# ksadov/FREUD

Hardware: AMD Instinct MI355X
Metric: SAE train activations/sec (d=384 dict 8x) (higher is better)
Workload: dtype bf16; 1 GPU; Whisper-tiny d=384 dict 8x (n=3072) L1 SAE train step, M=65536 rows/GPU/step, RAdam+cosine, x bfloat16 resident in HBM (BASELINE configs[1]); rows_per_gpu=65536, d_model=384, n_dict=3072, parallelism=dp1, dp=none

## Files before the change

### freud_amd/csrc/engine.hip

```cpp
#include <hip/hip_runtime.h>
#include <math.h>
#include <stdarg.h>
#include <stdio.h>
#include <string.h>

#include <algorithm>
#include <utility>
#include <vector>

#include "../../include/freud_sae.h"
#include "l1_kernels.h"
#include "gemm256.h"
#include "gemm256s.h"
#include "gemm256_fp8.h"
#include "l1_fp8.h"
#include "dp_kernels.h"
#include "p2p_exchange.h"
#include <rccl/rccl.h>
#include <mutex>
#include <unistd.h>

static thread_local bool g_force_gemm128 = false;
static thread_local bool g_no_stream = false;
static thread_local int g_device = 0;
// ... 67 lines not shown
  KID_PREP_X,
  KID_ENC_FWD,
  KID_DEC_FWD,
  KID_FWD_FUSED,
  KID_DPRE,
  KID_DW,
  KID_BWD_FUSED,
  KID_REDUCE,
  KID_OPT,
  KID_TK_ENC,
  KID_TK_SELECT,
  KID_TK_DECODE,
  KID_TK_DDENSE,
  KID_TK_DWD,
  KID_TK_DWE,
  KID_TK_DSAE,
  KID_TK_AUX,
  KID_EXCHANGE,
  KID_STATS_XCHG,
  KID_STEP_TOTAL,
  KID_COUNT
};
static const char* kKernelNames[KID_COUNT] = {"prep_w", "prep_x", "enc_fwd_gemm", "dec_fwd_gemm", "fwd_fused_gemm", "dpre_gemm",
                                              "dw_gemm", "bwd_fused_gemm", "reduce_grads", "clip_adam", "topk_enc_gemm", "topk_select",
                                              "topk_decode", "topk_ddense_gemm", "topk_dwdec_gemm", "topk_dwenc_gemm",
                                              "topk_dsaein_colsum", "topk_auxk_backward", "dp_exchange", "dp_stats_exchange",
                                              "fwd_bwd_total"};
constexpr int EV_RING = 64;

struct EvRing {
  hipEvent_t beg[EV_RING], end[EV_RING];
  int n = 0;
};

enum LastCall { LAST_FWD_BF16 = 0, LAST_FWD_E32, LAST_SEARCH, LAST_STATS };

struct sae_ctx {
  sae_config cfg;
  int d, n, d_p, n_p;
  int64_t max_rows_p;
  int64_t nW;
  int64_t nparams;
  float *P = nullptr, *Mom = nullptr, *Var = nullptr;
  float* G = nullptr;
  bf16_t *Wb = nullptr, *Wt = nullptr;
  bool fp8 = false;
  bool fp8_bwd = false;
  unsigned char* dxh8 = nullptr;
  int row_pad = 128;
  unsigned char *x8 = nullptr, *c8 = nullptr, *W8 = nullptr, *W8t = nullptr;
  float *scal8 = nullptr, *x8_part = nullptr;
  bool use_fused_fwd = false;
  int fwd_variant = 2;
  bf16_t *xb = nullptr, *c = nullptr, *dxh = nullptr, *dpre = nullptr;
  bf16_t *dxhT = nullptr, *xT = nullptr;
  float *slab = nullptr, *db_part = nullptr, *l1_part = nullptr, *sq_part = nullptr, *scal = nullptr;
  double* gn_part = nullptr;
  float* cn_part = nullptr;
  bool cn_valid = false;
  bool wb_valid = false;
  float* cnorm = nullptr;
  bool wn_pending = false, wn_fwd_seen = false;
  sae_grad_ready_fn grad_ready = nullptr;
  void* grad_ready_user = nullptr;
  int dw_chunk_rows = 0;
  int dw_chunk_splits = 1;
  int dw_col_chunks = 1;
  int dw_col_splits = 1;
  float* cnt_part = nullptr;
  int gn_blocks = 0;
  bool step_fused_call = false;
  bool gn_valid = false;
  bool metrics_fresh = false;
  const bf16_t* xb_cur = nullptr;
  unsigned int* masked = nullptr;
  int dw_splits = 1;
  int dw_tail_tiles = 0, dw_tail_pieces = 0;
  float* dw_tail = nullptr;
  int bwd_splits = 1;
  int bwd_range_splits = 1;
  bool use_fused_bwd = false;
  bool topk = false;
  int k = 0, k_aux_cap = 0;
  int64_t rows_per_file = 0;
  double dead_threshold = 1e300;
  bf16_t *We_b = nullptr, *Wd_b = nullptr, *xs = nullptr, *pre = nullptr, *dense = nullptr, *aux_dense = nullptr;
  bf16_t *de_b = nullptr, *dh_b = nullptr;
  float *e = nullptr, *dh = nullptr, *e2_part = nullptr, *a2_part = nullptr, *dbd_part = nullptr, *ds_part = nullptr, *tkf = nullptr;
  int *top_idx = nullptr, *aux_idx = nullptr, *tk = nullptr;
  bf16_t *top_vals = nullptr, *aux_vals = nullptr, *multi_vals = nullptr;
  unsigned short* tile_max = nullptr;
  unsigned char* sel_flag = nullptr;
  bool dense_valid = false;
  bool multi_dense_valid = false;
  float* be_r = nullptr;
  int slab_splits = 1;
  bool aux_compact = false;
  int *tkd = nullptr, *dead_cols = nullptr, *vec_rank = nullptr;
  unsigned char* vec_bits = nullptr;
  bf16_t* Wdd_b = nullptr;
  float* aux_dbe_part = nullptr;
  int* dead_hint = nullptr;
  double* tv_part = nullptr;
  long long* nfsf = nullptr;
  long long* dbe_fx = nullptr;
  bool topk_sparse_da = false;
// ... 342 lines not shown
    return fail(SAE_ERR_INVALID, "Invalid precision: %d, must be SAE_PREC_BF16, SAE_PREC_FP8 or SAE_PREC_FP8_BWD", cfg->precision);
  if (cfg->precision != SAE_PREC_BF16 && cfg->variant != SAE_VARIANT_L1)
    return fail(SAE_ERR_INVALID, "fp8 encoder / decoder GEMMs exist for the L1 variant only");

  sae_ctx* c = new sae_ctx();
  c->cfg = *cfg;
  c->d = cfg->d_model;
  c->n = cfg->n_dict;
  c->fp8 = cfg->precision != SAE_PREC_BF16;
  c->fp8_bwd = cfg->precision == SAE_PREC_FP8_BWD;
  const int pad = c->fp8 ? 256 : 128;
  c->row_pad = pad;
  c->d_p = (int)round_up(c->d, pad);
  c->n_p = (int)round_up(c->n, pad);
  c->max_rows_p = round_up(cfg->max_rows, pad);
  c->nW = (int64_t)c->d_p * c->n_p;
  c->nparams = c->nW + c->n_p;
  c->topk = cfg->variant == SAE_VARIANT_TOPK;
  if (const char* fg = getenv("FREUD_P2P_FINEGRAINED")) c->finegrained = atoi(fg) == 1;
  const int64_t Mp = c->max_rows_p;
  if (c->topk) {
    int rc_tk = topk_create(c, Mp);
    if (rc_tk) {
      sae_destroy(c);
      return rc_tk;
    }
    *out = c;
    return SAE_OK;
  }
  g_force_gemm128 = cfg->force_gemm128 == 1;
  c->no_stream = g_no_stream = cfg->debug_flags == 86 || (getenv("FREUD_GEMM_STREAM") && atoi(getenv("FREUD_GEMM_STREAM")) == 0);
  c->dw_splits = choose_splits(c->d_p / 128, c->n_p / 128, 2 * Mp / 64);
  if (const char* ov = getenv("FREUD_DW_SPLITS")) {
    const int v = atoi(ov);
    if (v >= 1 && v <= 64) c->dw_splits = v;
  }
  c->dw_chunk_rows = c->d_p >= 1024 ? 512 : c->d_p;
  if (!g_force_gemm128 && c->d_p % 256 == 0 && c->n_p % 256 == 0 && (c->d_p / 256) * (c->n_p / 256) >= 256 && !getenv("FREUD_DW_SPLITS") &&
      c->cfg.debug_flags != 81) {
    gemm_tail_plan((c->d_p / 256) * (c->n_p / 256), (int)(2 * Mp / 64), c->dw_tail_tiles, c->dw_tail_pieces);
    if ((c->d_p / 256) * (c->n_p / 256) % 256 == 0) c->dw_tail_tiles = c->dw_tail_pieces = -1;
  }
  c->dw_chunk_splits = choose_splits(c->dw_chunk_rows / 128, c->n_p / 128, 2 * Mp / 64);
  if (c->d_p >= 1024 && c->n_p % 256 == 0)
    for (int q = 4; q >= 2; --q)
      if ((c->n_p / 256) % q == 0) {
        c->dw_col_chunks = q;
        break;
      }
  c->dw_col_splits = choose_splits(c->d_p / 128, c->n_p / 128 / c->dw_col_chunks, 2 * Mp / 64);
  c->use_fused_bwd = (c->d_p == BF_D) && cfg->force_generic != 1 && !c->fp8;
  c->use_fused_fwd = (c->d_p == FF_D) && cfg->force_generic != 1 && !c->fp8;
  if (const char* fv = getenv("FREUD_FWD")) c->fwd_variant = atoi(fv) == 1 ? 1 : 2;
  c->bwd_splits = fused_bwd_splits(c->n_p / BF_BN, (int)(Mp / BF_BM), c->n_p);
  c->bwd_range_splits = c->bwd_splits;
  for (int r = 2; r <= 4; ++r)
    if ((c->n_p / BF_BN) % r == 0) {
      const int sp = fused_bwd_splits(c->n_p / BF_BN / r, (int)(Mp / BF_BM), c->n_p / r);
      if (sp > c->bwd_range_splits) c->bwd_range_splits = sp;
    }
  int slab_splits = c->use_fused_bwd ? (c->bwd_range_splits > c->dw_splits ? c->bwd_range_splits : c->dw_splits) : c->dw_splits;
  if (c->use_fused_bwd && c->cfg.debug_flags != 83 && !getenv("FREUD_BWD_UNIFORM")) {
    const int ntiles = c->n_p / BF_BN, cus = 256;
    const int m = (32 * ntiles + cus - 1) / cus, grid = (32 * ntiles + m - 1) / m;
    int pmax = 1;
    for (int j = 0; j < ntiles; ++j) pmax = bal_pieces(j, m) > pmax ? bal_pieces(j, m) : pmax;
    const int steps = (int)(Mp / BF_BM), q = (steps + 31) / 32;
    const double slab_steps = (double)c->n_p * BF_D * 8.0 / 4.0e12 / 1.43e-6;
    const double cost_bal = (double)m * q + 5.0 + (32 % m ? 3.5 : 0.0) + (32.0 / m + (32 % m ? 1.0 : 0.0)) * slab_steps;
    const int sp = c->bwd_splits, rounds = (ntiles * sp + 255) / 256;
    const double cost_uni = rounds * ((double)((steps + sp - 1) / sp) + 5.0) + sp * slab_steps;
    if (cost_bal < cost_uni * 0.995 && pmax <= 64 && grid <= 4096) {
      c->bal_m = m;
      c->bal_grid = grid;
      if (pmax > slab_splits) slab_splits = pmax;
      std::vector<int> order(grid);
      for (int k = 0; k < grid; ++k) order[k] = k;
      std::stable_sort(order.begin(), order.end(), [m](int a_, int b_) { return (a_ * m) % 32 < (b_ * m) % 32; });
      std::vector<short> map(grid);
      int pos = 0;
      for (int x = 0; x < 8; ++x) {
        const int len = grid / 8 + (x < grid % 8 ? 1 : 0);
        for (int i = 0; i < len; ++i) map[8 * i + x] = (short)order[pos++];
      }
      hipError_t e_ = hipMalloc((void**)&c->bal_map, (size_t)grid * 2);
      if (e_ == hipSuccess) e_ = hipMemcpy(c->bal_map, map.data(), (size_t)grid * 2, hipMemcpyHostToDevice);
      if (e_ != hipSuccess) {
        int rc_ = fail(SAE_ERR_HIP, "balanced backward: workgroup table: %s", hipGetErrorString(e_));
        sae_destroy(c);
        return rc_;
      }
    }
  }
  {
    const int64_t need = (int64_t)(c->dw_chunk_splits > c->dw_col_splits ? c->dw_chunk_splits : c->dw_col_splits);
    if (need > slab_splits) slab_splits = (int)need;
  }
  const int64_t db_rows = (Mp / 128) > 64 ? (Mp / 128) : 64;

#define ALLOC(ptr, bytes)                                   \
  do {                                                      \
    hipError_t e_ = hipMalloc((void**)&(ptr), (bytes));     \
    if (e_ != hipSuccess) {                                 \
      int rc_ = fail(SAE_ERR_HIP, "hipMalloc(%lld bytes) for %s failed: %s", (long long)(bytes), #ptr, \
                     hipGetErrorString(e_));                \
      sae_destroy(c);                                       \
// ... 889 lines not shown
template <typename T>
static int forward_impl(sae_ctx* c, const T* x, int64_t M, int64_t Mp, hipStream_t s, bool need_backward) {
  const int d = c->d, d_p = c->d_p, n_p = c->n_p;
  const float alpha = (float)c->cfg.recon_alpha;
  float* W = c->P;
  float* b = c->P + c->nW;

  ev_begin(c, KID_PREP_W, s);
  prep_weights_l1(c, s);
  if (c->fp8) hipLaunchKernelGGL(fp8_cast_w_kernel, dim3(n_p / 64, d_p / 64), dim3(256), 0, s, W, c->W8, c->W8t, d_p, n_p);
  ev_end(c, KID_PREP_W, s);

  ev_begin(c, KID_PREP_X, s);
  const bool alias_x = c->use_fused_fwd && sizeof(T) == 2 && x_dtype_is_bf16<T>() && d == d_p && M == Mp &&
                       (reinterpret_cast<uintptr_t>(x) & 15) == 0;
  c->xb_cur = alias_x ? reinterpret_cast<const bf16_t*>(x) : c->xb;
  if (!alias_x) {
    const int grid = launch_prep_x(c, x, M, Mp, s);
    if (!c->use_fused_fwd) {
      const double* gs = (need_backward && c->dp_world > 0) ? c->stats : nullptr;
      if (gs && c->dist) HIP_TRY(hipStreamWaitEvent(s, c->ev_stats, 0));
      hipLaunchKernelGGL(finalize_count_kernel, dim3(1), dim3(256), 0, s, c->masked, grid, c->scal, M, d, alpha, gs);
    }
  }
  if (c->fp8) {
    const int sgrid = (int)((Mp / 4) < 1024 ? (Mp / 4) : 1024);
    hipLaunchKernelGGL(fp8_x_stats_kernel, dim3(sgrid), dim3(256), 0, s, c->xb, Mp, d_p, c->x8_part);
    hipLaunchKernelGGL(fp8_scales_kernel, dim3(1), dim3(256), 0, s, c->x8_part, sgrid, b, c->n, c->scal8);
    const int64_t n8 = Mp * (d_p / 8);
    hipLaunchKernelGGL(fp8_quant_x_kernel, dim3(grid_for(n8, 2048)), dim3(256), 0, s, c->xb, c->x8, n8, c->scal8);
  }
  ev_end(c, KID_PREP_X, s);

  int rc;
  if (c->use_fused_fwd) {
    const int lds = FF_LDS_BYTES;
    FwdFusedArgs a{};
    a.xb = c->xb_cur; a.x = x; a.Wt = c->Wt; a.bias = b; a.cnt_part = c->cnt_part; a.c = c->c; a.dxh = c->dxh;
    a.l1_part = c->l1_part; a.sq_part = c->sq_part; a.M = M; a.d = d; a.n_p = n_p; a.ntiles = n_p / FF_BN;
    a.c_rows = c->max_rows_p;
    const int full_wgs = (int)(M / FF_BM), all_wgs = (int)(Mp / FF_BM);
    auto launch = [&](auto kern, int blocks, int block_offset) -> int {
      LDS_ATTR(kern, 160 * 1024, g_device);
      a.block_offset = block_offset;
      hipLaunchKernelGGL(kern, dim3(blocks), dim3(256), lds, s, a);
      return SAE_OK;
    };
    ev_begin(c, KID_FWD_FUSED, s);
    int rcl = SAE_OK;
    if (full_wgs > 0 && c->cfg.debug_flags == 65 && c->fwd_variant == 1) {
      a.stamps = reinterpret_cast<unsigned long long*>(c->dpre);
      rcl = launch(fwd_fused_d384_kernel<T, false, true>, full_wgs, 0);
    } else if (c->fwd_variant == 2) {
      if (full_wgs > 0 && c->cfg.debug_flags == 65) {
        a.stamps = reinterpret_cast<unsigned long long*>(c->dpre);
        rcl = launch(fwd_fused2_d384_kernel<T, false, true>, full_wgs, 0);
      } else if (full_wgs > 0) rcl = launch(fwd_fused2_d384_kernel<T, false>, full_wgs, 0);
      if (!rcl && all_wgs > full_wgs) rcl = launch(fwd_fused2_d384_kernel<T, true>, all_wgs - full_wgs, full_wgs);
      if (rcl) return rcl;
      ev_end(c, KID_FWD_FUSED, s);
      HIP_TRY(hipGetLastError());
      return SAE_OK;
    } else if (full_wgs > 0) {
      rcl = launch(fwd_fused_d384_kernel<T, false, false>, full_wgs, 0);
    }
    if (!rcl && all_wgs > full_wgs) rcl = launch(fwd_fused_d384_kernel<T, true, false>, all_wgs - full_wgs, full_wgs);
    if (rcl) return rcl;
    ev_end(c, KID_FWD_FUSED, s);
    HIP_TRY(hipGetLastError());
    return SAE_OK;
  }
  if (c->fp8) {
    {
      Gemm8Args g{};
      g.A = c->x8; g.B = c->W8t; g.lda = d_p; g.ldb = d_p;
      g.nbm = (int)(Mp / 256); g.nbn = n_p / 256; g.ktiles = d_p / 128;
      EpiEnc8 e{};
      e.c = c->c; e.c8 = c->c8; e.bias = b; e.scal8 = c->scal8; e.l1_part = c->l1_part; e.M = M; e.n_p = n_p; e.nbn = n_p / 128;
      if (gemm8_streams<EpiEnc8>(g)) HIP_TRY(hipMemsetAsync(c->l1_part, 0, (size_t)(Mp / 128) * (n_p / 128) * 4, s));
      ev_begin(c, KID_ENC_FWD, s);
      rc = launch_gemm8(g, e, s);
      ev_end(c, KID_ENC_FWD, s);
      if (rc) return rc;
    }
    {
      Gemm8Args g{};
      g.A = c->c8; g.B = c->W8; g.lda = n_p; g.ldb = n_p;
      g.nbm = (int)(Mp / 256); g.nbn = d_p / 256; g.ktiles = n_p / 128;
      EpiDec<T> e{};
      e.x = x; e.dxh = c->dxh; e.scal = c->scal; e.sq_part = c->sq_part; e.M = M; e.d = d; e.d_p = d_p; e.nbn = d_p / 128;
      e.vec_all = (M == Mp && d == d_p && d % 4 == 0 && (reinterpret_cast<uintptr_t>(x) % (4 * sizeof(T))) == 0) ? 1 : 0;
      e.vscale = c->scal8 + S8_INV_DEC;
      ev_begin(c, KID_DEC_FWD, s);
      rc = launch_gemm8(g, e, s);
      ev_end(c, KID_DEC_FWD, s);
      if (rc) return rc;
    }
    if (need_backward && c->dxhT) {
      hipLaunchKernelGGL(transpose_bf16_kernel, dim3((unsigned)(Mp / 64), d_p / 64), dim3(256), 0, s, c->dxh, c->dxhT, Mp, d_p);
      hipLaunchKernelGGL(transpose_bf16_kernel, dim3((unsigned)(Mp / 64), d_p / 64), dim3(256), 0, s, c->xb_cur, c->xT, Mp, d_p);
      HIP_TRY(hipGetLastError());
    }
    return SAE_OK;
  }
  rc = launch_encoder<T>(c, enc_gemm_args(c, c->xb_cur, Mp), M, s);
  if (rc) return rc;
  {
    GemmArgs g{};
    g.A0 = c->c; g.B0 = c->Wb; g.lda = n_p; g.ldb = n_p;
    g.nbm = (int)(Mp / 128); g.nbn = d_p / 128; g.ktiles0 = g.ktiles = n_p / 64; g.splits = 1;
// ... 1447 lines not shown
```

### freud_amd/csrc/fwd_fused2.h

```cpp
#pragma once
#include "fwd_fused.h"

typedef __attribute__((ext_vector_type(2))) float f32x2_t;

template <typename T, bool PAD, bool STAMP = false>
__global__ __launch_bounds__(256, 1) void fwd_fused2_d384_kernel(FwdFusedArgs a) {
  extern __shared__ __attribute__((aligned(16))) char smem[];
  const int t = threadIdx.x, lane = t & 63, w = t >> 6;
  const int arow = lane & 31, ah = lane >> 5;
  const int wg = blockIdx.x + a.block_offset;
  const int64_t m0 = (int64_t)wg * FF_BM + 32 * w;
  const int64_t mrow = m0 + arow;
  const bool row_ok = mrow < a.M;
  char* cst = smem + FF_RING_BYTES;
  float* bias_s = reinterpret_cast<float*>(smem + FF_FIXED_LDS);
  unsigned long long clk_k0 = 0, clk_t0 = 0, clk_r0 = 0, clk_t1 = 0;
  if (STAMP) clk_k0 = __builtin_amdgcn_s_memtime();

  typedef __attribute__((ext_vector_type(2))) unsigned short us2_t;
  constexpr unsigned MASK_BITS2 = std::is_same<T, bf16_t>::value ? 0xBF80BF80u : 0xBC00BC00u;
  constexpr bool SCAN_EARLY = !PAD && std::is_same<T, bf16_t>::value;
  bool wany_early = false;

  bf16x8 xfrag[24];
  unsigned voff_t[6], loff_t[6];
#pragma unroll
  for (int i = 0; i < 6; ++i) {
    const int inst = w + 4 * i, sub = inst >> 3, row = 4 * (inst & 7) + (lane >> 4), pc = lane & 15;
    const int ch = pc ^ (((row & 3) << 2) | ((row >> 2) & 3));
    voff_t[i] = (unsigned)(row * (FF_D * 2) + (sub * 16 + ch) * 16);
    loff_t[i] = (unsigned)__builtin_amdgcn_readfirstlane(sub * 8192 + (inst & 7) * 1024);
  }
  typedef __attribute__((address_space(3))) char* lptr_t;
  const unsigned smem_base = (unsigned)(uintptr_t)(lptr_t)smem;
  auto dma_pair = [&](int p, int jt, int st) {
    const bf16_t* src = a.Wt + (int64_t)jt * FF_BN * FF_D;
    const unsigned dst = smem_base + st * FF_WT_BYTES;
    glds16_x2(src, src, voff_t[2 * p], voff_t[2 * p + 1], (unsigned)__builtin_amdgcn_readfirstlane((int)(dst + loff_t[2 * p])),
              (unsigned)__builtin_amdgcn_readfirstlane((int)(dst + loff_t[2 * p + 1])));
  };
  auto dma_one = [&](int k, int jt, int st) {
    const bf16_t* src = a.Wt + (int64_t)jt * FF_BN * FF_D;
    glds16(src, voff_t[k], (unsigned)__builtin_amdgcn_readfirstlane((int)(smem_base + st * FF_WT_BYTES + loff_t[k])));
  };
  const int last = a.ntiles - 1;
#pragma unroll
  for (int q = 0; q < 3; ++q)
#pragma unroll
    for (int p = 0; p < 3; ++p) dma_pair(p, q <= last ? q : last, q);
  static_assert(2 * FF_BN == 64, "one 4-byte piece per lane of wave 0");
  if (w == 0) glds4(a.bias, (unsigned)(lane * 4), (unsigned)__builtin_amdgcn_readfirstlane((int)(smem_base + FF_FIXED_LDS)));
  {
    const bf16_t* xp = a.xb + mrow * FF_D + 8 * ah;
#pragma unroll
    for (int kk = 0; kk < 24; ++kk) xfrag[kk] = *reinterpret_cast<const bf16x8*>(xp + 16 * kk);
  }
  for (int i = t; i < FF_WT_BYTES / 16; i += 256) reinterpret_cast<u32x4*>(smem + 3 * FF_WT_BYTES)[i] = u32x4{0u, 0u, 0u, 0u};
  for (int i = t; i < FF_CST_BYTES / 16; i += 256) reinterpret_cast<u32x4*>(cst)[i] = u32x4{0u, 0u, 0u, 0u};

  f32x16 acc[12];
#pragma unroll
  for (int i = 0; i < 12; ++i)
#pragma unroll
    for (int r = 0; r < 16; ++r) acc[i][r] = 0.f;

  if (SCAN_EARLY) {
    us2_t mz = {0xFFFFu, 0xFFFFu};
#pragma unroll
    for (int kk = 0; kk < 24; ++kk) {
      const u32x4 xw = __builtin_bit_cast(u32x4, xfrag[kk]);
#pragma unroll
      for (int c = 0; c < 4; ++c) mz = __builtin_elementwise_min(mz, __builtin_bit_cast(us2_t, xw[c] ^ MASK_BITS2));
    }
    wany_early = __builtin_amdgcn_ballot_w64((mz[0] == 0) | (mz[1] == 0)) != 0ull;
  }
#pragma unroll
  for (int kk = 0; kk < 24; ++kk) asm volatile("" : "+v"(xfrag[kk]));
  asm volatile("s_waitcnt vmcnt(0)" ::: "memory");
  __syncthreads();

  int roff[8];
#pragma unroll
  for (int i = 0; i < 8; ++i) roff[i] = dual_off(arow, 2 * i + ah);
  int aoff0[6], aoff1[6];
  {
    const int g = (lane >> 4) & 1, q = (lane & 15) >> 2, p = lane & 3;
#pragma unroll
    for (int f = 0; f < 6; ++f) {
      const int ks = f / 3, dt = 3 * w + f % 3;
      const int col = 32 * (dt & 3) + 16 * g + 4 * p;
      const int r0 = 4 * ah + q, r1 = r0 + 8;
      const int base = (dt >> 2) * 8192 + ks * 4096;
      aoff0[f] = base + dual_off(r0, col >> 3) + (col & 7) * 2;
      aoff1[f] = base + dual_off(r1, col >> 3) + (col & 7) * 2;
    }
  }
  typedef __attribute__((ext_vector_type(8))) short s16x8;
  auto tr_pair = [&](const char* p0, const char* p1) -> bf16x8 {
    const s16x4 lo = __builtin_amdgcn_ds_read_tr16_b64_v4i16(LDS_PTR(s16x4, p0));
    const s16x4 hi = __builtin_amdgcn_ds_read_tr16_b64_v4i16(LDS_PTR(s16x4, p1));
    const s16x8 v = __builtin_shufflevector(lo, hi, 0, 1, 2, 3, 4, 5, 6, 7);
    return __builtin_bit_cast(bf16x8, v);
  };
  auto swz = [](int row) { return (row & 7) ^ ((row >> 1) & 1) ^ ((row >> 4) & 1); };
  int boff[4];
#pragma unroll
  for (int i = 0; i < 4; ++i) boff[i] = arow * 128 + (((4 * (i >> 1) + 2 * (i & 1) + ah) ^ swz(arow)) << 4);
  const int wrow = w * 4096;
  const int drow_l = lane >> 3, dch = lane & 7;
  int doff0, doff1;
  {
    const int tl = dch >> 2, s = (dch & 3) >> 1, u = dch & 1;
    doff0 = drow_l * 128 + (((4 * tl + 2 * s + 0) ^ swz(drow_l)) << 4) + 8 * u;
    doff1 = drow_l * 128 + (((4 * tl + 2 * s + 1) ^ swz(drow_l)) << 4) + 8 * u;
  }
  auto dpiece = [](int off, int p) { return (p & 2) ? (off ^ 16) : off; };
  bf16_t* cdrain = a.c + (m0 + drow_l) * a.n_p + dch * 8;

  float l1_acc = 0.f;

  f32x16 Sn;
#pragma unroll
  for (int r = 0; r < 16; ++r) Sn[r] = 0.f;
#pragma unroll
  for (int kk = 0; kk < 24; ++kk) {
    const bf16x8 fa = *reinterpret_cast<const bf16x8*>(smem + (kk >> 3) * 8192 + roff[kk & 7]);
    Sn = __builtin_amdgcn_mfma_f32_32x32x16_bf16(fa, xfrag[kk], Sn, 0, 0, 0);
  }

  constexpr int RING = 8;
  const char *rlo[8], *rhi[8];
#pragma unroll
  for (int i = 0; i < 8; ++i) {
// ... 93 lines not shown
      if (i == 41 || i == 45) dma_one((i - 41) / 4, jt, SLOT_DMA);
      if (i == 1 || i == 5 || i == 9 || i == 13) dma_one(2 + (i - 1) / 4, j + 2 <= last ? j + 2 : last, (PH + 2) & 3);
      if ((PH & 1) == 0 && i == 46 && w == 0) {
        const int jb = j + 2 <= a.ntiles - 2 ? j + 2 : a.ntiles - 2;
        glds4(a.bias + (int64_t)jb * FF_BN, (unsigned)(lane * 4),
              (unsigned)__builtin_amdgcn_readfirstlane((int)(smem_base + FF_FIXED_LDS + ((j + 2) & (FF_BIAS_RING_TILES - 1)) * FF_BN * 4)));
      }
      if (i >= 4 && i <= 35) {
        const int p = (i - 4) >> 2, ph = (i - 4) & 3, e0 = 2 * p;
        if (ph == 0) {
          se_u = __builtin_bit_cast(unsigned, __builtin_convertvector(f32x2_t{S[e0], S[e0 + 1]}, bf16x2));
        } else if (ph == 1) {
          se_t0 = __uint_as_float(se_u << 16) + bq[e0 >> 2][e0 & 3];
          se_t1 = __uint_as_float(se_u & 0xFFFF0000u);
        } else if (ph == 2) {
          se_t1 = se_t1 + bq[e0 >> 2][(e0 & 3) + 1];
          se_t0 = fmaxf(se_t0, 0.f);
          se_t1 = fmaxf(se_t1, 0.f);
          if (PAD) { se_t0 = row_ok ? se_t0 : 0.f; se_t1 = row_ok ? se_t1 : 0.f; }
        } else {
          asm volatile("v_add_f32 %0, %0, %1\n\tv_add_f32 %0, %0, %2" : "+v"(l1_it) : "v"(se_t0), "v"(se_t1));
          cw[e0 & 7] = (bf16_t)se_t0;
          cw[(e0 & 7) + 1] = (bf16_t)se_t1;
          if ((e0 & 7) == 6)
            *reinterpret_cast<bf16x8*>(cst + PB_W * 16384 + wrow + boff[2 * HF_W + (e0 >> 3)]) = cw;
        }
      }
      if (i == 29 || i == 33) {
        const int p = 2 * (PH & 1) + (i == 33);
        const uint2 lo = *reinterpret_cast<const uint2*>(cst_r + p * 1024 + dpiece(doff0, p));
        const uint2 hi = *reinterpret_cast<const uint2*>(cst_r + p * 1024 + dpiece(doff1, p));
        dr[i == 33] = u32x4{lo.x, lo.y, hi.x, hi.y};
      }
      if (i == 37 || i == 42) {
        const int p = 2 * (PH & 1) + (i == 42);
        __builtin_nontemporal_store(dr[i == 42], reinterpret_cast<u32x4*>(dst_pair + (int64_t)(8 * p) * dst_rstride));
      }
      __builtin_amdgcn_sched_barrier(0);
      if ((i & 1) == 0) {
        const int m = i / 2, ks = m / 12, mb = (m % 12) / 3, dtl = m % 3;
        acc[4 * dtl + mb] = __builtin_amdgcn_mfma_f32_32x32x16_bf16(Afr[3 * ks + dtl], Bq[(4 * ks + mb) & 3], acc[4 * dtl + mb], 0, 0, 0);
      } else if (i == 1) {
        f32x16 zero;
#pragma unroll
        for (int r = 0; r < 16; ++r) zero[r] = 0.f;
        Snxt = __builtin_amdgcn_mfma_f32_32x32x16_bf16(ring[0], xfrag[0], zero, 0, 0, 0);
      } else {
        Snxt = __builtin_amdgcn_mfma_f32_32x32x16_bf16(ring[(i / 2) % RING], xfrag[i / 2], Snxt, 0, 0, 0);
      }
      __builtin_amdgcn_sched_barrier(0);
    });
    l1_acc += l1_it + 0.0f;
  };
  if (STAMP) { clk_t0 = __builtin_amdgcn_s_memtime(); clk_r0 = __builtin_amdgcn_s_memrealtime(); }
  for (int j4 = 0; j4 < a.ntiles; j4 += 4) {
    body(std::integral_constant<int, 0>{}, j4);
    body(std::integral_constant<int, 1>{}, j4 + 1);
    body(std::integral_constant<int, 2>{}, j4 + 2);
    body(std::integral_constant<int, 3>{}, j4 + 3);
  }
  if (STAMP) {
    const unsigned long long t1 = __builtin_amdgcn_s_memtime(), r1 = __builtin_amdgcn_s_memrealtime();
    clk_t1 = t1;
    if (lane == 0) {
      unsigned long long* o = a.stamps + ((int64_t)wg * 4 + w) * 8;
      o[0] = o[1] = o[2] = 0; o[3] = (unsigned long long)a.ntiles; o[4] = t1 - clk_t0; o[5] = r1 - clk_r0; o[6] = clk_t0 - clk_k0;
    }
  }
  Bq[2] = dec_b(1, 1, 2);
#pragma unroll
  for (int m = 0; m < 24; ++m) {
    if (m == 3 || m == 4 || m == 5) Afr[m] = dec_a(3, m);
    if (m % 3 == 0 && m / 3 + 3 <= 7) Bq[(m / 3 + 3) & 3] = dec_b(1, 1, m / 3 + 3);
    __builtin_amdgcn_sched_barrier(0);
    const int ks = m / 12, mb = (m % 12) / 3, dtl = m % 3;
    acc[4 * dtl + mb] = __builtin_amdgcn_mfma_f32_32x32x16_bf16(Afr[3 * ks + dtl], Bq[(4 * ks + mb) & 3], acc[4 * dtl + mb], 0, 0, 0);
    __builtin_amdgcn_sched_barrier(0);
  }
  {
    const char* cst_r = cst + (((a.ntiles >> 1) - 1) & 1) * 16384 + wrow;
#pragma unroll
    for (int p = 0; p < 4; ++p) {
      const uint2 lo = *reinterpret_cast<const uint2*>(cst_r + p * 1024 + dpiece(doff0, p));
      const uint2 hi = *reinterpret_cast<const uint2*>(cst_r + p * 1024 + dpiece(doff1, p));
      __builtin_nontemporal_store(u32x4{lo.x, lo.y, hi.x, hi.y},
                                  reinterpret_cast<u32x4*>(cdrain + (int64_t)(8 * p) * a.n_p + 64 * ((a.ntiles >> 1) - 1)));
    }
  }
  __builtin_amdgcn_sched_barrier(0);
  asm volatile("s_waitcnt vmcnt(4) lgkmcnt(0)" ::: "memory");
  __builtin_amdgcn_s_barrier();
  __builtin_amdgcn_sched_barrier(0);

  unsigned long long clk_e0 = 0, clk_e1 = 0, clk_e2 = 0;
  if (STAMP) clk_e0 = __builtin_amdgcn_s_memtime();
  float sq = 0.f, plain = 0.f, nmask = 0.f;
  float msq = 0.f;
  f32x2_t plain2 = {0.f, 0.f};
  typedef __attribute__((ext_vector_type(4))) T Tx4;
  const bool vec_ok = (a.d == FF_D) && ((reinterpret_cast<uintptr_t>(a.x) & (sizeof(T) * 4 - 1)) == 0);
  constexpr int FF_DXH_PITCH = FF_D * 2 + 16;
  static_assert(128 * FF_DXH_PITCH <= FF_FIXED_LDS, "the dx_hat staging must fit the idle LDS");
  char* stg = smem;
  constexpr bool X_VIA_LDS = !PAD && sizeof(T) == 2;
  constexpr bool X_FROM_FRAGS = X_VIA_LDS && std::is_same<T, bf16_t>::value;
  unsigned* mflag = reinterpret_cast<unsigned*>(smem + FF_FIXED_LDS + 64);
  bool blk_masked = true;
  if (X_FROM_FRAGS && vec_ok && reinterpret_cast<const void*>(a.x) == reinterpret_cast<const void*>(a.xb)) {
    char* srow_w = stg + (32 * w + arow) * FF_DXH_PITCH + 16 * ah;
    us2_t mz = {0xFFFFu, 0xFFFFu};
#pragma unroll
    for (int kk = 0; kk < 24; ++kk) {
      *reinterpret_cast<bf16x8*>(srow_w + 32 * kk) = xfrag[kk];
      if (!SCAN_EARLY) {
        const u32x4 xw = __builtin_bit_cast(u32x4, xfrag[kk]);
#pragma unroll
        for (int c = 0; c < 4; ++c) mz = __builtin_elementwise_min(mz, __builtin_bit_cast(us2_t, xw[c] ^ MASK_BITS2));
      }
    }
    const bool wany = SCAN_EARLY ? wany_early : __builtin_amdgcn_ballot_w64((mz[0] == 0) | (mz[1] == 0)) != 0ull;
    if (lane == 0) mflag[w] = wany ? 1u : 0u;
    __syncthreads();
    const u32x4 f = *reinterpret_cast<const u32x4*>(mflag);
    blk_masked = (f[0] | f[1] | f[2] | f[3]) != 0u;
  } else
  if (X_VIA_LDS && vec_ok) {
    const char* xblk = reinterpret_cast<const char*>(reinterpret_cast<const T*>(a.x) + m0 * FF_D);
    us2_t mz = {0xFFFFu, 0xFFFFu};
#pragma unroll
    for (int p0 = 0; p0 < 24; p0 += 4) {
      u32x4 xr[4];
#pragma unroll
      for (int pc = 0; pc < 4; ++pc) xr[pc] = *reinterpret_cast<const u32x4*>(xblk + (p0 + pc) * 1024 + lane * 16);
#pragma unroll
      for (int pc = 0; pc < 4; ++pc) {
        const int off = (p0 + pc) * 1024 + lane * 16, r = off / (FF_D * 2), cb = off - r * (FF_D * 2);
        *reinterpret_cast<u32x4*>(stg + (32 * w + r) * FF_DXH_PITCH + cb) = xr[pc];
#pragma unroll
        for (int c = 0; c < 4; ++c) mz = __builtin_elementwise_min(mz, __builtin_bit_cast(us2_t, xr[pc][c] ^ MASK_BITS2));
      }
    }
    const bool wany = __builtin_amdgcn_ballot_w64((mz[0] == 0) | (mz[1] == 0)) != 0ull;
    if (lane == 0) mflag[w] = wany ? 1u : 0u;
    __syncthreads();
    const u32x4 f = *reinterpret_cast<const u32x4*>(mflag);
    blk_masked = (f[0] | f[1] | f[2] | f[3]) != 0u;
  }
  if (STAMP) clk_e1 = __builtin_amdgcn_s_memtime();
  auto residual = [&](auto notest_tag) {
  constexpr bool NOTEST = decltype(notest_tag)::value;
  constexpr bool FENCE = NOTEST && X_VIA_LDS;
  constexpr bool PIPE = FENCE && std::is_same<T, bf16_t>::value;
  Tx4 xq[2][4];
  auto xload = [&](int g, Tx4 (&dst)[4]) {
    const char* sr = stg + (32 * (g / 3) + arow) * FF_DXH_PITCH + (96 * w + 32 * (g % 3) + 4 * ah) * 2;
#pragma unroll
    for (int k = 0; k < 4; ++k) dst[k] = *reinterpret_cast<const Tx4*>(sr + 16 * k);
  };
  if constexpr (PIPE) xload(0, xq[0]);
#pragma unroll
  for (int mb = 0; mb < 4; ++mb) {
    const int64_t grow = (int64_t)wg * FF_BM + 32 * mb + arow;
    const bool ok = !PAD || grow < a.M;
    const float rmask = ok ? 1.f : 0.f;
    const T* xrow = reinterpret_cast<const T*>(a.x) + (ok ? grow : a.M - 1) * a.d;
    char* srow = stg + (32 * mb + arow) * FF_DXH_PITCH;
#pragma unroll
    for (int dtl = 0; dtl < 3; ++dtl) {
      const int dbase = 96 * w + 32 * dtl + 4 * ah;
      if (NOTEST || vec_ok) {
        const int g = 3 * mb + dtl;
        if constexpr (FENCE) {
          if (g > 0) __builtin_amdgcn_sched_barrier(0);
          if (PIPE && g + 1 < 12) xload(g + 1, xq[(g + 1) & 1]);
        }
        Tx4 xv[4];
#pragma unroll
        for (int k = 0; k < 4; ++k)
          xv[k] = PIPE ? xq[g & 1][k]
                       : (X_VIA_LDS ? *reinterpret_cast<const Tx4*>(srow + (dbase + 8 * k) * 2) : *reinterpret_cast<const Tx4*>(xrow + dbase + 8 * k));
        if (!PAD) {
          if constexpr (NOTEST && X_VIA_LDS) {
            if constexpr (std::is_same<T, bf16_t>::value) {
              uint2 ow[4];
#pragma unroll
              for (int k = 0; k < 4; ++k) {
                const uint2 xw = __builtin_bit_cast(uint2, xv[k]);
#pragma unroll
                for (int pp = 0; pp < 2; ++pp) {
                  const unsigned xd = pp ? xw.y : xw.x;
                  const unsigned rb = __builtin_bit_cast(unsigned, __builtin_convertvector(
                      f32x2_t{acc[4 * dtl + mb][4 * k + 2 * pp], acc[4 * dtl + mb][4 * k + 2 * pp + 1]}, bf16x2));
                  const f32x2_t rf = {__uint_as_float(rb << 16), __uint_as_float(rb & 0xFFFF0000u)};
                  const f32x2_t xf = {__uint_as_float(xd << 16), __uint_as_float(xd & 0xFFFF0000u)};
                  f32x2_t e2, d2;
                  asm("v_pk_add_f32 %0, %1, %2 neg_lo:[0,1] neg_hi:[0,1]" : "=v"(e2) : "v"(rf), "v"(xf));
                  asm("v_pk_fma_f32 %0, %1, %1, %0" : "+v"(plain2) : "v"(e2));
                  asm("v_pk_add_f32 %0, %1, %1" : "=v"(d2) : "v"(e2));
                  const unsigned ob = __builtin_bit_cast(unsigned, __builtin_convertvector(d2, bf16x2));
                  if (pp) ow[k].y = ob; else ow[k].x = ob;
                }
// ... 26 lines not shown
              const float e = bf16_round(acc[4 * dtl + mb][4 * k + q]) - xf;
              const bool mk = xf == -1.0f;
              const float em = mk ? e : 0.0f, ek = mk ? 0.0f : e;
              plain = __builtin_fmaf(e, e, plain);
              msq = __builtin_fmaf(em, em, msq);
              nm_i += mk ? 1u : 0u;
              o[k][q] = (bf16_t)(ek + ek);
            }
          nmask += (float)nm_i;
#pragma unroll
          for (int k = 0; k < 4; ++k) *reinterpret_cast<bf16x4*>(srow + (dbase + 8 * k) * 2) = o[k];
          continue;
        }
#pragma unroll
        for (int k = 0; k < 4; ++k) {
          bf16x4 o;
#pragma unroll
          for (int q = 0; q < 4; ++q) {
            const float xf = (float)xv[k][q];
            const float e = bf16_round(acc[4 * dtl + mb][4 * k + q]) - xf;
            const float e2 = e * e;
            plain += rmask * e2;
            const float keep = (xf != -1.0f) ? rmask : 0.f;
            nmask += rmask - keep;
            sq += keep * e2;
            o[q] = (bf16_t)(keep * (e * 2.0f));
          }
          *reinterpret_cast<bf16x4*>(srow + (dbase + 8 * k) * 2) = o;
        }
      } else {
#pragma unroll
        for (int k = 0; k < 4; ++k) {
          bf16x4 o;
#pragma unroll
          for (int q = 0; q < 4; ++q) {
            const int dd = dbase + 8 * k + q;
            const bool valid = dd < a.d;
            const float xf = (float)xrow[valid ? dd : a.d - 1];
            const float e = bf16_round(acc[4 * dtl + mb][4 * k + q]) - xf;
            const float e2 = valid ? e * e : 0.f;
            plain += rmask * e2;
            const float keep = (valid && xf != -1.0f) ? rmask : 0.f;
            nmask += (valid ? rmask : 0.f) - keep;
            sq += keep * e2;
            o[q] = (bf16_t)(keep * (e * 2.0f));
          }
          *reinterpret_cast<bf16x4*>(srow + (dbase + 8 * k) * 2) = o;
        }
      }
    }
  }
  };
  if (X_VIA_LDS && vec_ok && !blk_masked) residual(std::true_type{}); else residual(std::false_type{});
  if (STAMP) clk_e2 = __builtin_amdgcn_s_memtime();
  __syncthreads();
  {
    char* gblk = reinterpret_cast<char*>(a.dxh + m0 * FF_D);
#pragma unroll
    for (int pc = 0; pc < 24; ++pc) {
      const int off = pc * 1024 + lane * 16, r = off / (FF_D * 2), cb = off - r * (FF_D * 2);
      *reinterpret_cast<u32x4*>(gblk + off) = *reinterpret_cast<const u32x4*>(stg + (32 * w + r) * FF_DXH_PITCH + cb);
    }
  }
  plain += plain2[0] + plain2[1];
  if (!PAD && vec_ok) sq = plain - msq;
  float* red = reinterpret_cast<float*>(smem + FF_FIXED_LDS);
  {
    const float v0 = wave_sum(l1_acc), v1 = wave_sum(sq), v2 = wave_sum(plain), v3 = wave_sum(nmask);
    if (lane == 0) *reinterpret_cast<f32x4*>(red + 4 * w) = f32x4{v0, v1, v2, v3};
  }
  lds_barrier();
  const float l1s = ((red[0] + red[4]) + red[8]) + red[12];
  const float sqs = ((red[1] + red[5]) + red[9]) + red[13];
  const float pls = ((red[2] + red[6]) + red[10]) + red[14];
  const float nms = ((red[3] + red[7]) + red[11]) + red[15];
  if (STAMP && lane == 0) {
    unsigned long long* o = a.stamps + ((int64_t)wg * 4 + w) * 8;
    const unsigned long long te = __builtin_amdgcn_s_memtime();
    o[7] = te - clk_k0;
    o[0] = clk_e0 - clk_t1; o[1] = clk_e1 - clk_e0; o[2] = clk_e2 - clk_e1;
#ifdef FF2_WAITSTAMP
    o[0] = ws_vm; o[1] = ws_bar; o[2] = ws_gap;
#endif
  }
  if (t == 0) {
    a.cnt_part[wg] = nms;
    a.l1_part[wg] = l1s;
    a.sq_part[2 * wg] = sqs;
    a.sq_part[2 * wg + 1] = pls;
  }
}
```

Before: 120.5 million activations/s.

## Make fused d384 forward kernel persistent with early prefetch of next block's x

Changes the bf16 fused forward kernel into a persistent grid of about one workgroup per CU that walks row blocks with a stride, instead of launching one workgroup per 128-row block. During the epilogue of each block it issues the x-fragment loads for the next block, overlapping global loads with the residual computation. It also moves the reduction scratch to a separate LDS offset and swaps some __syncthreads for LDS-only barriers. This removes per-workgroup launch and prologue cost, but it re-streams the W tiles for every block, raises register pressure from the prefetched fragments, and may unbalance the tail.

Measured after the change: 120.6 million activations/s (median of 2 runs). About the same (+0.1%).

```diff
diff --git a/freud_amd/csrc/engine.hip b/freud_amd/csrc/engine.hip
--- a/freud_amd/csrc/engine.hip
+++ b/freud_amd/csrc/engine.hip
@@ -143,6 +143,8 @@
   float *scal8 = nullptr, *x8_part = nullptr;
   bool use_fused_fwd = false;
   int fwd_variant = 2;
+  int fwd_cus = 256;
+  int fwd_wgs = 0;
   bf16_t *xb = nullptr, *c = nullptr, *dxh = nullptr, *dpre = nullptr;
   bf16_t *dxhT = nullptr, *xT = nullptr;
   float *slab = nullptr, *db_part = nullptr, *l1_part = nullptr, *sq_part = nullptr, *scal = nullptr;
@@ -591,6 +593,11 @@
   c->use_fused_bwd = (c->d_p == BF_D) && cfg->force_generic != 1 && !c->fp8;
   c->use_fused_fwd = (c->d_p == FF_D) && cfg->force_generic != 1 && !c->fp8;
   if (const char* fv = getenv("FREUD_FWD")) c->fwd_variant = atoi(fv) == 1 ? 1 : 2;
+  {
+    int cus = 0;
+    if (hipDeviceGetAttribute(&cus, hipDeviceAttributeMultiprocessorCount, cfg->device_id) == hipSuccess && cus > 0) c->fwd_cus = cus;
+    if (const char* fw = getenv("FREUD_FWD_WGS")) c->fwd_wgs = atoi(fw) > 0 ? atoi(fw) : 0;
+  }
   c->bwd_splits = fused_bwd_splits(c->n_p / BF_BN, (int)(Mp / BF_BM), c->n_p);
   c->bwd_range_splits = c->bwd_splits;
   for (int r = 2; r <= 4; ++r)
@@ -1586,10 +1593,13 @@
       a.stamps = reinterpret_cast<unsigned long long*>(c->dpre);
       rcl = launch(fwd_fused_d384_kernel<T, false, true>, full_wgs, 0);
     } else if (c->fwd_variant == 2) {
+      int G = full_wgs < c->fwd_cus ? full_wgs : c->fwd_cus;
+      if (G < full_wgs && G > 8) G -= G % 8;
+      if (c->fwd_wgs > 0) G = c->fwd_wgs < full_wgs ? c->fwd_wgs : full_wgs;
       if (full_wgs > 0 && c->cfg.debug_flags == 65) {
         a.stamps = reinterpret_cast<unsigned long long*>(c->dpre);
         rcl = launch(fwd_fused2_d384_kernel<T, false, true>, full_wgs, 0);
-      } else if (full_wgs > 0) rcl = launch(fwd_fused2_d384_kernel<T, false>, full_wgs, 0);
+      } else if (full_wgs > 0) rcl = launch(fwd_fused2_d384_kernel<T, false>, ff2_persistent<T, false, false> ? G : full_wgs, 0);
       if (!rcl && all_wgs > full_wgs) rcl = launch(fwd_fused2_d384_kernel<T, true>, all_wgs - full_wgs, full_wgs);
       if (rcl) return rcl;
       ev_end(c, KID_FWD_FUSED, s);
diff --git a/freud_amd/csrc/fwd_fused2.h b/freud_amd/csrc/fwd_fused2.h
--- a/freud_amd/csrc/fwd_fused2.h
+++ b/freud_amd/csrc/fwd_fused2.h
@@ -2,19 +2,27 @@
 #include "fwd_fused.h"
 
 typedef __attribute__((ext_vector_type(2))) float f32x2_t;
+
+template <typename T, bool PAD, bool STAMP>
+constexpr bool ff2_persistent = !PAD && !STAMP && (std::is_same<T, bf16_t>::value || sizeof(T) == 4);
 
 template <typename T, bool PAD, bool STAMP = false>
 __global__ __launch_bounds__(256, 1) void fwd_fused2_d384_kernel(FwdFusedArgs a) {
   extern __shared__ __attribute__((aligned(16))) char smem[];
   const int t = threadIdx.x, lane = t & 63, w = t >> 6;
   const int arow = lane & 31, ah = lane >> 5;
-  const int wg = blockIdx.x + a.block_offset;
-  const int64_t m0 = (int64_t)wg * FF_BM + 32 * w;
-  const int64_t mrow = m0 + arow;
+  constexpr bool PERSIST = ff2_persistent<T, PAD, STAMP>;
+  constexpr bool EARLY_X = PERSIST;
+  int wg = blockIdx.x + a.block_offset;
+  const int wg_step = PERSIST ? (int)gridDim.x : 0;
+  const int wg_end = PERSIST ? (int)(a.M / FF_BM) : 0;
+  int64_t m0 = (int64_t)wg * FF_BM + 32 * w;
+  int64_t mrow = m0 + arow;
   const bool row_ok = mrow < a.M;
   char* cst = smem + FF_RING_BYTES;
   float* bias_s = reinterpret_cast<float*>(smem + FF_FIXED_LDS);
-  unsigned long long clk_k0 = 0, clk_t0 = 0, clk_r0 = 0, clk_t1 = 0;
+  unsigned clk_t0 = 0, clk_r0 = 0, clk_t1 = 0;
+  unsigned long long clk_k0 = 0;
   if (STAMP) clk_k0 = __builtin_amdgcn_s_memtime();
 
   typedef __attribute__((ext_vector_type(2))) unsigned short us2_t;
@@ -44,27 +52,23 @@
     glds16(src, voff_t[k], (unsigned)__builtin_amdgcn_readfirstlane((int)(smem_base + st * FF_WT_BYTES + loff_t[k])));
   };
   const int last = a.ntiles - 1;
-#pragma unroll
-  for (int q = 0; q < 3; ++q)
-#pragma unroll
-    for (int p = 0; p < 3; ++p) dma_pair(p, q <= last ? q : last, q);
-  static_assert(2 * FF_BN == 64, "one 4-byte piece per lane of wave 0");
-  if (w == 0) glds4(a.bias, (unsigned)(lane * 4), (unsigned)__builtin_amdgcn_readfirstlane((int)(smem_base + FF_FIXED_LDS)));
-  {
+  auto dma_first_tiles = [&]() {
+#pragma unroll
+    for (int q = 0; q < 3; ++q)
+#pragma unroll
+      for (int p = 0; p < 3; ++p) dma_pair(p, q <= last ? q : last, q);
+    if (w == 0) glds4(a.bias, (unsigned)(lane * 4), (unsigned)__builtin_amdgcn_readfirstlane((int)(smem_base + FF_FIXED_LDS)));
+  };
+  auto load_x = [&]() {
     const bf16_t* xp = a.xb + mrow * FF_D + 8 * ah;
 #pragma unroll
     for (int kk = 0; kk < 24; ++kk) xfrag[kk] = *reinterpret_cast<const bf16x8*>(xp + 16 * kk);
-  }
-  for (int i = t; i < FF_WT_BYTES / 16; i += 256) reinterpret_cast<u32x4*>(smem + 3 * FF_WT_BYTES)[i] = u32x4{0u, 0u, 0u, 0u};
-  for (int i = t; i < FF_CST_BYTES / 16; i += 256) reinterpret_cast<u32x4*>(cst)[i] = u32x4{0u, 0u, 0u, 0u};
-
-  f32x16 acc[12];
-#pragma unroll
-  for (int i = 0; i < 12; ++i)
-#pragma unroll
-    for (int r = 0; r < 16; ++r) acc[i][r] = 0.f;
-
-  if (SCAN_EARLY) {
+  };
+  auto zero_fill = [&]() {
+    for (int i = t; i < FF_WT_BYTES / 16; i += 256) reinterpret_cast<u32x4*>(smem + 3 * FF_WT_BYTES)[i] = u32x4{0u, 0u, 0u, 0u};
+    for (int i = t; i < FF_CST_BYTES / 16; i += 256) reinterpret_cast<u32x4*>(cst)[i] = u32x4{0u, 0u, 0u, 0u};
+  };
+  auto scan_x = [&]() -> bool {
     us2_t mz = {0xFFFFu, 0xFFFFu};
 #pragma unroll
     for (int kk = 0; kk < 24; ++kk) {
@@ -72,13 +76,29 @@
 #pragma unroll
       for (int c = 0; c < 4; ++c) mz = __builtin_elementwise_min(mz, __builtin_bit_cast(us2_t, xw[c] ^ MASK_BITS2));
     }
-    wany_early = __builtin_amdgcn_ballot_w64((mz[0] == 0) | (mz[1] == 0)) != 0ull;
-  }
+    return __builtin_amdgcn_ballot_w64((mz[0] == 0) | (mz[1] == 0)) != 0ull;
+  };
+  static_assert(2 * FF_BN == 64, "one 4-byte piece per lane of wave 0");
+  f32x16 acc[12];
+  constexpr int FF_RED_OFF = FF_FIXED_LDS + 2 * FF_BN * 4;
+  bool walking = false;
+  for (;;) {
+  dma_first_tiles();
+  if (!walking || !EARLY_X) load_x();
+  zero_fill();
+#pragma unroll
+  for (int i = 0; i < 12; ++i)
+#pragma unroll
+    for (int r = 0; r < 16; ++r) acc[i][r] = 0.f;
+  if (SCAN_EARLY) wany_early = scan_x();
 #pragma unroll
   for (int kk = 0; kk < 24; ++kk) asm volatile("" : "+v"(xfrag[kk]));
   asm volatile("s_waitcnt vmcnt(0)" ::: "memory");
   __syncthreads();
-
+  const bool has_next = PERSIST && wg + wg_step < wg_end;
+  int t_blk = t;
+  asm volatile("" : "+v"(t_blk));
+  const int lane = t_blk & 63, w = t_blk >> 6, arow = lane & 31, ah = lane >> 5;
   int roff[8];
 #pragma unroll
   for (int i = 0; i < 8; ++i) roff[i] = dual_off(arow, 2 * i + ah);
@@ -278,7 +298,13 @@
     });
     l1_acc += l1_it + 0.0f;
   };
-  if (STAMP) { clk_t0 = __builtin_amdgcn_s_memtime(); clk_r0 = __builtin_amdgcn_s_memrealtime(); }
+  if (STAMP) {
+    clk_t0 = (unsigned)__builtin_amdgcn_s_memtime(); clk_r0 = (unsigned)__builtin_amdgcn_s_memrealtime();
+    if (lane == 0) {
+      unsigned long long* o = a.stamps + ((int64_t)wg * 4 + w) * 8;
+      o[6] = clk_t0 - (unsigned)clk_k0; o[7] = 0ull - clk_k0;
+    }
+  }
   for (int j4 = 0; j4 < a.ntiles; j4 += 4) {
     body(std::integral_constant<int, 0>{}, j4);
     body(std::integral_constant<int, 1>{}, j4 + 1);
@@ -286,11 +312,11 @@
     body(std::integral_constant<int, 3>{}, j4 + 3);
   }
   if (STAMP) {
-    const unsigned long long t1 = __builtin_amdgcn_s_memtime(), r1 = __builtin_amdgcn_s_memrealtime();
+    const unsigned t1 = (unsigned)__builtin_amdgcn_s_memtime(), r1 = (unsigned)__builtin_amdgcn_s_memrealtime();
     clk_t1 = t1;
     if (lane == 0) {
       unsigned long long* o = a.stamps + ((int64_t)wg * 4 + w) * 8;
-      o[0] = o[1] = o[2] = 0; o[3] = (unsigned long long)a.ntiles; o[4] = t1 - clk_t0; o[5] = r1 - clk_r0; o[6] = clk_t0 - clk_k0;
+      o[0] = o[1] = o[2] = 0; o[3] = (unsigned long long)a.ntiles; o[4] = t1 - clk_t0; o[5] = r1 - clk_r0;
     }
   }
   Bq[2] = dec_b(1, 1, 2);
@@ -318,8 +344,12 @@
   __builtin_amdgcn_s_barrier();
   __builtin_amdgcn_sched_barrier(0);
 
-  unsigned long long clk_e0 = 0, clk_e1 = 0, clk_e2 = 0;
-  if (STAMP) clk_e0 = __builtin_amdgcn_s_memtime();
+  {
+  int t_epi = t;
+  asm volatile("" : "+v"(t_epi));
+  const int t = t_epi, lane = t & 63, w = t >> 6, arow = lane & 31, ah = lane >> 5;
+  unsigned clk_e0 = 0, clk_e1 = 0, clk_e2 = 0;
+  if (STAMP) clk_e0 = (unsigned)__builtin_amdgcn_s_memtime();
   float sq = 0.f, plain = 0.f, nmask = 0.f;
   float msq = 0.f;
   f32x2_t plain2 = {0.f, 0.f};
@@ -332,6 +362,13 @@
   constexpr bool X_FROM_FRAGS = X_VIA_LDS && std::is_same<T, bf16_t>::value;
   unsigned* mflag = reinterpret_cast<unsigned*>(smem + FF_FIXED_LDS + 64);
   bool blk_masked = true;
+  bool x_issued = false;
+  auto next_x = [&]() {
+    mrow += (int64_t)wg_step * FF_BM;
+    load_x();
+    asm volatile("" ::: "memory");
+    __builtin_amdgcn_sched_barrier(0);
+  };
   if (X_FROM_FRAGS && vec_ok && reinterpret_cast<const void*>(a.x) == reinterpret_cast<const void*>(a.xb)) {
     char* srow_w = stg + (32 * w + arow) * FF_DXH_PITCH + 16 * ah;
     us2_t mz = {0xFFFFu, 0xFFFFu};
@@ -346,7 +383,8 @@
     }
     const bool wany = SCAN_EARLY ? wany_early : __builtin_amdgcn_ballot_w64((mz[0] == 0) | (mz[1] == 0)) != 0ull;
     if (lane == 0) mflag[w] = wany ? 1u : 0u;
-    __syncthreads();
+    if (EARLY_X && has_next) { next_x(); x_issued = true; }
+    lds_barrier();
     const u32x4 f = *reinterpret_cast<const u32x4*>(mflag);
     blk_masked = (f[0] | f[1] | f[2] | f[3]) != 0u;
   } else
@@ -368,11 +406,11 @@
     }
     const bool wany = __builtin_amdgcn_ballot_w64((mz[0] == 0) | (mz[1] == 0)) != 0ull;
     if (lane == 0) mflag[w] = wany ? 1u : 0u;
-    __syncthreads();
+    lds_barrier();
     const u32x4 f = *reinterpret_cast<const u32x4*>(mflag);
     blk_masked = (f[0] | f[1] | f[2] | f[3]) != 0u;
   }
-  if (STAMP) clk_e1 = __builtin_amdgcn_s_memtime();
+  if (STAMP) clk_e1 = (unsigned)__builtin_amdgcn_s_memtime();
   auto residual = [&](auto notest_tag) {
   constexpr bool NOTEST = decltype(notest_tag)::value;
   constexpr bool FENCE = NOTEST && X_VIA_LDS;
@@ -505,8 +543,9 @@
   }
   };
   if (X_VIA_LDS && vec_ok && !blk_masked) residual(std::true_type{}); else residual(std::false_type{});
-  if (STAMP) clk_e2 = __builtin_amdgcn_s_memtime();
-  __syncthreads();
+  if (STAMP) clk_e2 = (unsigned)__builtin_amdgcn_s_memtime();
+  if (EARLY_X && has_next && !x_issued) next_x();
+  lds_barrier();
   {
     char* gblk = reinterpret_cast<char*>(a.dxh + m0 * FF_D);
 #pragma unroll
@@ -517,7 +556,7 @@
   }
   plain += plain2[0] + plain2[1];
   if (!PAD && vec_ok) sq = plain - msq;
-  float* red = reinterpret_cast<float*>(smem + FF_FIXED_LDS);
+  float* red = reinterpret_cast<float*>(smem + FF_RED_OFF);
   {
     const float v0 = wave_sum(l1_acc), v1 = wave_sum(sq), v2 = wave_sum(plain), v3 = wave_sum(nmask);
     if (lane == 0) *reinterpret_cast<f32x4*>(red + 4 * w) = f32x4{v0, v1, v2, v3};
@@ -527,19 +566,29 @@
   const float sqs = ((red[1] + red[5]) + red[9]) + red[13];
   const float pls = ((red[2] + red[6]) + red[10]) + red[14];
   const float nms = ((red[3] + red[7]) + red[11]) + red[15];
-  if (STAMP && lane == 0) {
-    unsigned long long* o = a.stamps + ((int64_t)wg * 4 + w) * 8;
-    const unsigned long long te = __builtin_amdgcn_s_memtime();
-    o[7] = te - clk_k0;
-    o[0] = clk_e0 - clk_t1; o[1] = clk_e1 - clk_e0; o[2] = clk_e2 - clk_e1;
-#ifdef FF2_WAITSTAMP
-    o[0] = ws_vm; o[1] = ws_bar; o[2] = ws_gap;
-#endif
-  }
   if (t == 0) {
     a.cnt_part[wg] = nms;
     a.l1_part[wg] = l1s;
     a.sq_part[2 * wg] = sqs;
     a.sq_part[2 * wg + 1] = pls;
   }
+  if (STAMP) {
+    const unsigned long long te = __builtin_amdgcn_s_memtime();
+    if (lane == 0) {
+      unsigned long long* o = a.stamps + ((int64_t)wg * 4 + w) * 8;
+      __hip_atomic_fetch_add(&o[7], te, __ATOMIC_RELAXED, __HIP_MEMORY_SCOPE_AGENT);
+      o[0] = clk_e0 - clk_t1; o[1] = clk_e1 - clk_e0; o[2] = clk_e2 - clk_e1;
+#ifdef FF2_WAITSTAMP
+      o[0] = ws_vm; o[1] = ws_bar; o[2] = ws_gap;
+#endif
+    }
+    clk_k0 = te;
+  }
+  }
+  if (!has_next) break;
+  wg += wg_step;
+  m0 += (int64_t)wg_step * FF_BM;
+  if (!EARLY_X) mrow += (int64_t)wg_step * FF_BM;
+  walking = true;
+  }
 }
```
